# bioinfo-pf-curie/mpiBWA

Hardware: AMD Instinct MI355X
Metric: Mreads/s (whole node) 2x150 bp PE vs GRCh38-size reference; SAM bit-match (higher is better)
Workload: dtype int32

## Files before the change

mpibwa_amd/csrc/msw_kernel.hip:

```cpp
#include <hip/hip_runtime.h>
#include <type_traits>
#include "hip_util.h"
#include "device.h"

namespace mbw {

namespace {

#define MSW_PAD 7u

__device__ __forceinline__ int msw_base(const uint8_t *__restrict__ pac, int64_t l_pac, int64_t p)
{
	if (p >= l_pac) {
		int64_t f = (l_pac << 1) - 1 - p;
		return 3 - ((pac[f >> 2] >> ((~f & 3) << 1)) & 3);
	}
	return (pac[p >> 2] >> ((~p & 3) << 1)) & 3;
}

struct MswPassOut { int score, te, qe; };

#define MSW_QP(a, b, c, d) ((a) | (b) << 2 | (c) << 4 | (d) << 6)
template <int CTRL>
__device__ __forceinline__ int msw_dpp(int v) { return __builtin_amdgcn_update_dpp(0, v, CTRL, 0xf, 0xf, false); }

__device__ __forceinline__ uint32_t msw_code(const uint8_t *__restrict__ ms, int qlen, int is_rev, int k)
{
	if (k >= qlen) return MSW_PAD;
	if (is_rev) { const uint32_t b = ms[qlen - 1 - k]; return b < 4 ? 3 - b : 4; }
	const uint32_t c = ms[k];
	return c > 4 ? 4 : c;
}

__device__ __forceinline__ MswPassOut msw_pass(uint32_t *cell, const MswParams &P, const uint8_t *__restrict__ pac, bool live, int S, int tn,
                                               int64_t t0, int tdir, int endsc, int sat_limit, uint16_t *rows, size_t row_stride, int *sat_hit)
{
	const int lane = threadIdx.x, j = lane & 3;
	int gmax = 0, te = -1, qe = -1;
	bool run = live && tn > 0 && S > 0;
	const int oe_del = P.o_del + P.e_del, oe_ins = P.o_ins + P.e_ins, e_del = P.e_del, e_ins = P.e_ins;
	int Swave = run ? S : 0;
	for (int o = 32; o; o >>= 1) Swave = max(Swave, __shfl_xor(Swave, o));
	int co_diag = 0, co_fseg = 0, co_ffull = 0, co_key = 0;
	int tb_next = (run && j == 0) ? msw_base(pac, P.l_pac, t0) : 0;
	for (int t = 0; __any(run); ++t) {
		const int i = t - j;
		const bool act = run && i >= 0 && i < tn;
		const int tb = tb_next;
		if (run && i + 1 >= 0 && i + 1 < tn) tb_next = msw_base(pac, P.l_pac, t0 + (int64_t)(i + 1) * tdir);
		const uint32_t slo = tb == 0 ? P.slo[0] : tb == 1 ? P.slo[1] : tb == 2 ? P.slo[2] : P.slo[3];
		const uint32_t shi = (uint32_t)(uint8_t)(tb == 0 ? P.s4[0] : tb == 1 ? P.s4[1] : tb == 2 ? P.s4[2] : P.s4[3]);
		const int ci_diag = msw_dpp<MSW_QP(0, 0, 1, 2)>(co_diag), ci_fseg = msw_dpp<MSW_QP(0, 0, 1, 2)>(co_fseg);
		const int ci_ffull = msw_dpp<MSW_QP(0, 0, 1, 2)>(co_ffull), ci_key = msw_dpp<MSW_QP(0, 0, 1, 2)>(co_key);
		int diag = j ? ci_diag : 0, fseg = j ? ci_fseg : 0, ffull = j ? ci_ffull : 0;
		uint32_t key = j ? (uint32_t)ci_key : 0u;
		const int kbase = j * S;
		const int kmax = act ? S : 0;
		auto step = [&](uint32_t &w, int kk) {
			const int hk = w & 0x1fff;
			int e = (int)__builtin_amdgcn_ubfe(w, 13, 13);
			const uint32_t q = __builtin_amdgcn_ubfe(w, 26, 3);
			const int s = (int)(int8_t)__builtin_amdgcn_perm(shi, slo, q | 0x0c0c0c00u);
			const int h = max(max(diag + s, e), fseg);
			key = max(key, (uint32_t)h << 16 | (uint32_t)(0xffff - (kbase + kk)));
			const int hfin = max(h, ffull);
			e = max(max(e - e_del, h - oe_del), 0);
			const int t2 = h - oe_ins;
			fseg = max(max(fseg - e_ins, t2), 0);
			ffull = max(max(ffull - e_ins, t2), 0);
			fseg &= ~((int)w >> 31);
			diag = hk;
			w = (w & 0xfc000000u) | ((uint32_t)e << 13 | (uint32_t)hfin);
		};
		for (int k = 0; k < Swave; k += 2) {
			if (k < kmax) {
				uint32_t w0 = cell[k * 64 + lane], w1 = cell[(k + 1) * 64 + lane];
				step(w0, k); step(w1, k + 1);
				cell[k * 64 + lane] = w0; cell[(k + 1) * 64 + lane] = w1;
			}
		}
		if (act) { co_diag = diag; co_fseg = fseg; co_ffull = ffull; co_key = (int)key; }
		int stop = 0;
		if (act && j == 3) {
			const int imax = (int)(key >> 16);
			if (rows) rows[(size_t)i * row_stride] = (uint16_t)imax;
			if (imax > gmax) {
				gmax = imax; te = i; qe = 0xffff - (int)(key & 0xffff);
				if (gmax >= sat_limit) { *sat_hit = 1; stop = 1; }
				if (gmax >= endsc) stop = 1;
			}
			if (i + 1 >= tn) stop = 1;
		}
		stop = msw_dpp<MSW_QP(3, 3, 3, 3)>(stop);
		if (stop) run = false;
	}
	MswPassOut o;
	o.score = msw_dpp<MSW_QP(3, 3, 3, 3)>(gmax); o.te = msw_dpp<MSW_QP(3, 3, 3, 3)>(te); o.qe = msw_dpp<MSW_QP(3, 3, 3, 3)>(qe);
	*sat_hit = msw_dpp<MSW_QP(3, 3, 3, 3)>(*sat_hit);
	return o;
}

__device__ __forceinline__ void msw_tail(uint32_t *cell, const MswParams &P, const uint8_t *__restrict__ pac, bool live, const MswReq &rq, int qlen,
                                         const uint8_t *__restrict__ ms, int r, int n_req, MswPassOut f, int sat, uint16_t *__restrict__ rows,
                                         MswRes *__restrict__ res)
{
	const int lane = threadIdx.x, j = lane & 3;
	const int tlen = (int)(rq.re - rq.rb);
	const bool byte_flavour = qlen * P.a < 250;
	const int PP = byte_flavour ? 16 : 8;
	const int minsc = P.min_seed_len * P.a;
	const int sat_limit = byte_flavour ? 255 - P.shift : 0x10000;
	MswRes out;
	out.score = f.score; out.te = f.te; out.qe = f.qe; out.score2 = -1; out.te2 = -1; out.tb = -1; out.qb = -1; out.flags = sat;
	if (live && j == 0 && !sat && f.te >= 0 && f.score >= minsc) {
		const int d = (f.score + P.max_sc - 1) / P.max_sc;
		const int low = f.te - d, high = f.te + d;
		int last_sc = -1, last_i = -1;
		const int rows_done = f.te >= 0 ? tlen : 0;
		for (int i = 0; i < rows_done; ++i) {
			const int im = rows[(size_t)i * n_req + r];
			if (im < minsc) continue;
			if (last_i < 0 || last_i + 1 != i) {
				if (last_i >= 0 && (last_i < low || last_i > high) && last_sc > out.score2) { out.score2 = last_sc; out.te2 = last_i; }
				last_sc = im; last_i = i;
			} else if (last_sc < im) { last_sc = im; last_i = i; }
		}
		if (last_i >= 0 && (last_i < low || last_i > high) && last_sc > out.score2) { out.score2 = last_sc; out.te2 = last_i; }
	}
	const bool second = live && !sat && f.score >= minsc && f.qe >= 0 && f.te >= 0;
	int qlen2 = second ? f.qe + 1 : 0;
	if (second && f.qe >= qlen) qlen2 = 0;
	const int slen2 = (qlen2 + PP - 1) / PP, npos2 = slen2 * PP, S2 = npos2 >> 2;
	if (qlen2 > 0)
		for (int kk = 0; kk < S2; ++kk) {
			const int k = j * S2 + kk;
			const uint32_t c = k < qlen2 ? msw_code(ms, qlen, rq.is_rev, qlen2 - 1 - k) : MSW_PAD;
			cell[kk * 64 + lane] = c << 26 | ((k + 1) % slen2 == 0 ? 0x80000000u : 0u);
		}
	int sat2 = 0;
	MswPassOut g = msw_pass(cell, P, pac, qlen2 > 0, S2, f.te + 1, rq.rb + f.te, -1, f.score, sat_limit, nullptr, 0, &sat2);
	if (qlen2 > 0 && g.score == f.score) { out.tb = f.te - g.te; out.qb = f.qe - g.qe; }
	if (second && qlen2 == 0) out.flags = 1;
	if (sat2) out.flags = 1;
	if (live && j == 0) res[r] = out;
}

__global__ __launch_bounds__(64) void msw_kernel(MswParams P, int n_work, int n_req, const int *__restrict__ list, const MswReq *__restrict__ req,
                                                 const uint8_t *__restrict__ seq, const int64_t *__restrict__ off, const int *__restrict__ lens,
                                                 const uint8_t *__restrict__ pac, MswRes *__restrict__ res, uint16_t *__restrict__ rows)
{
	extern __shared__ uint32_t cell[];
	const int lane = threadIdx.x, j = lane & 3;
	const int slot = blockIdx.x * 16 + (lane >> 2);
	const bool live = slot < n_work;
	const int r = live ? (list ? list[slot] : slot) : 0;
	MswReq rq;
	rq.rb = rq.re = 0; rq.read = 0; rq.is_rev = 0;
	if (live) rq = req[r];
	const int qlen = live ? lens[rq.read] : 0;
	const int tlen = (int)(rq.re - rq.rb);
	const bool byte_flavour = qlen * P.a < 250;
	const int PP = byte_flavour ? 16 : 8;
	const int slen = (qlen + PP - 1) / PP;
	const int npos = slen * PP, S = npos >> 2;
	const uint8_t *ms = seq + (live ? off[rq.read] : 0);
	if (live)
		for (int kk = 0; kk < S; ++kk) {
			const int k = j * S + kk;
			cell[kk * 64 + lane] = msw_code(ms, qlen, rq.is_rev, k) << 26 | ((k + 1) % slen == 0 ? 0x80000000u : 0u);
		}
	const int sat_limit = byte_flavour ? 255 - P.shift : 0x10000;
	int sat = 0;
	MswPassOut f = msw_pass(cell, P, pac, live, S, tlen, rq.rb, 1, 0x10000, sat_limit, live ? rows + r : nullptr, (size_t)n_req, &sat);
	msw_tail(cell, P, pac, live, rq, qlen, ms, r, n_req, f, sat, rows, res);
}

typedef short msw_s2 __attribute__((ext_vector_type(2)));
__device__ __forceinline__ msw_s2 s2_of(uint32_t v) { return __builtin_bit_cast(msw_s2, v); }
__device__ __forceinline__ uint32_t u_of(msw_s2 v) { return __builtin_bit_cast(uint32_t, v); }
__device__ __forceinline__ msw_s2 s2_max(msw_s2 a, msw_s2 b) { return __builtin_elementwise_max(a, b); }
__device__ __forceinline__ msw_s2 s2_splat(int v) { msw_s2 r; r.x = (short)v; r.y = (short)v; return r; }
typedef unsigned short msw_u2 __attribute__((ext_vector_type(2)));
__device__ __forceinline__ msw_s2 s2_sub0(msw_s2 a, msw_s2 b)
{
	return __builtin_bit_cast(msw_s2, __builtin_elementwise_sub_sat(__builtin_bit_cast(msw_u2, a), __builtin_bit_cast(msw_u2, b)));
}

__device__ __forceinline__ int msw_tail_bucket(int score, int qe, int a)
{
	const int sb = score >= 80 * a ? 2 : score >= 40 * a ? 1 : 0;
	const int qb = qe >= 96 ? 2 : qe >= 48 ? 1 : 0;
	return sb * 3 + qb;
}

__device__ __forceinline__ uint32_t msw_slo(const MswParams &P, int t) { return t == 0 ? P.slo[0] : t == 1 ? P.slo[1] : t == 2 ? P.slo[2] : P.slo[3]; }
__device__ __forceinline__ int msw_s4(const MswParams &P, int t) { return t == 0 ? P.s4[0] : t == 1 ? P.s4[1] : t == 2 ? P.s4[2] : P.s4[3]; }

__global__ __launch_bounds__(64) void msw2_kernel(MswParams P, int n_pairs, int n_req, const int *__restrict__ pairs, const MswReq *__restrict__ req,
                                                  const uint8_t *__restrict__ seq, const int64_t *__restrict__ off, const int *__restrict__ lens,
                                                  const uint8_t *__restrict__ pac, MswRes *__restrict__ res, uint16_t *__restrict__ rows, int s_max,
                                                  int *__restrict__ tail_n, int *__restrict__ tail_list, int tail_cap)
{
	extern __shared__ uint32_t lds2[];
	uint32_t *cell = lds2;
	uint32_t *codes = lds2 + (size_t)s_max * 64;
	uint32_t *stab = codes + (size_t)((s_max + 7) >> 3) * 64;
	const int lane = threadIdx.x, j = lane & 3;
	for (int e = lane; e < 128; e += 64) {
		const int ta = e >> 5, tb = (e >> 3) & 3, q = e & 7;
		const int sa = q < 4 ? (int)(int8_t)(msw_slo(P, ta) >> (8 * q)) : q == 4 ? msw_s4(P, ta) : 0;
		const int sb = q < 4 ? (int)(int8_t)(msw_slo(P, tb) >> (8 * q)) : q == 4 ? msw_s4(P, tb) : 0;
		stab[e] = (uint32_t)(uint16_t)(int16_t)sa | (uint32_t)(uint16_t)(int16_t)sb << 16;
	}
	const int slot = blockIdx.x * 16 + (lane >> 2);
	const bool live = slot < n_pairs;
	const int rA = live ? pairs[2 * slot] : 0, rB = live ? pairs[2 * slot + 1] : -1;
	const bool hasB = rB >= 0;
	MswReq qa, qb;
	qa.rb = qa.re = 0; qa.read = 0; qa.is_rev = 0; qb = qa;
	if (live) { qa = req[rA]; if (hasB) qb = req[rB]; else { qb = qa; qb.re = qb.rb; } }
	const int qlen = live ? lens[qa.read] : 0;
	const int tnA = (int)(qa.re - qa.rb), tnB = (int)(qb.re - qb.rb);
	const int slen = (qlen + 15) / 16, npos = slen * 16, S = npos >> 2;
	const uint8_t *ms = seq + (live ? off[qa.read] : 0);
	if (live) {
		for (int kk = 0; kk < S; ++kk) cell[kk * 64 + lane] = 0;
		for (int c = 0; c * 8 < S; ++c) {
			uint32_t cd = 0;
			for (int u = 0; u < 8 && c * 8 + u < S; ++u) {
				const int k = j * S + c * 8 + u;
				cd |= (msw_code(ms, qlen, qa.is_rev, k) | ((k + 1) % slen == 0 ? 8u : 0u)) << (4 * u);
			}
			codes[c * 64 + lane] = cd;
		}
	}
	__builtin_amdgcn_fence(__ATOMIC_RELEASE, "wavefront");
	__builtin_amdgcn_wave_barrier();
	__builtin_amdgcn_fence(__ATOMIC_ACQUIRE, "wavefront");
	const int sat_limit = 255 - P.shift;
	int slen_u = 0;
	{
		const unsigned long long lv = __builtin_amdgcn_ballot_w64(live);
		if (lv) {
			const int first = __builtin_amdgcn_readlane(slen, __ffsll((long long)lv) - 1);
			slen_u = __builtin_amdgcn_ballot_w64(live && slen != first) ? 0 : first;
		}
	}
	int gmaxA = 0, teA = -1, qeA = -1, gmaxB = 0, teB = -1, qeB = -1, satA = 0, satB = 0;
	auto forward = [&](auto uniform_segments) {
		constexpr bool UNI = decltype(uniform_segments)::value;
		const int tn = tnA > tnB ? tnA : tnB;
		bool run = live && tn > 0 && S > 0;
		const msw_s2 oe_del = s2_splat(P.o_del + P.e_del), oe_ins = s2_splat(P.o_ins + P.e_ins), e_del = s2_splat(P.e_del), e_ins = s2_splat(P.e_ins);
		const msw_s2 zero = s2_splat(0);
		int Swave = run ? S : 0;
		for (int o = 32; o; o >>= 1) Swave = max(Swave, __shfl_xor(Swave, o));
		uint32_t co_diag = 0, co_fseg = 0, co_ffull = 0, co_key = 0;
		auto base_at = [&](const MswReq &rq, int tnx, int i) -> int {
			const int ii = i < tnx ? i : tnx - 1;
			return ii >= 0 ? msw_base(pac, P.l_pac, rq.rb + ii) : 0;
		};
		int ta_next = (run && j == 0) ? base_at(qa, tnA, 0) : 0, tb_next = (run && j == 0) ? base_at(qb, tnB, 0) : 0;
		uint16_t *rowsA = rows + rA, *rowsB = rows + (hasB ? rB : rA);
		for (int t = 0; __any(run); ++t) {
			const int i = t - j;
			const bool act = run && i >= 0 && i < tn;
			const int ta = ta_next, tb = tb_next;
			if (run && i + 1 >= 0 && i + 1 < tn) { ta_next = base_at(qa, tnA, i + 1); tb_next = base_at(qb, tnB, i + 1); }
			const uint32_t *srow = stab + ((ta << 2 | tb) << 3);
			const uint32_t ci_diag = (uint32_t)msw_dpp<MSW_QP(0, 0, 1, 2)>((int)co_diag), ci_fseg = (uint32_t)msw_dpp<MSW_QP(0, 0, 1, 2)>((int)co_fseg);
			const uint32_t ci_ffull = (uint32_t)msw_dpp<MSW_QP(0, 0, 1, 2)>((int)co_ffull);
			const uint32_t ci_key = (uint32_t)msw_dpp<MSW_QP(0, 0, 1, 2)>((int)co_key);
			msw_s2 diag = s2_of(j ? ci_diag : 0u), fseg = s2_of(j ? ci_fseg : 0u), ffull = s2_of(j ? ci_ffull : 0u);
			msw_u2 key = __builtin_bit_cast(msw_u2, j ? ci_key : 0u);
			msw_u2 c256 = {256, 256};
			asm volatile("" : "+v"(c256));
			msw_u2 poscv = {(unsigned short)(248 - j * S), (unsigned short)(248 - j * S)};
			const int kmax = act ? S : 0;
			auto step = [&](uint32_t &w, uint32_t cd, int u, bool seg_end, msw_u2 &mblk) {
				const msw_s2 hd = s2_of(__builtin_amdgcn_perm(0u, w, 0x0c020c00u));
				msw_s2 e = s2_of(__builtin_amdgcn_perm(0u, w, 0x0c030c01u));
				uint32_t q = __builtin_amdgcn_ubfe(cd, 4 * u, 3);
				asm("" : "+v"(q));
				const msw_s2 s = s2_of(srow[q]);
				const msw_s2 h = s2_max(s2_max(diag + s, e), fseg);
				const msw_u2 rel = {(unsigned short)(7 - u), (unsigned short)(7 - u)};
				mblk = __builtin_elementwise_max(mblk, __builtin_bit_cast(msw_u2, h) * c256 + rel);
				const msw_s2 hfin = s2_max(h, ffull);
				e = s2_max(s2_sub0(e, e_del), s2_sub0(h, oe_del));
				const msw_s2 t2 = s2_sub0(h, oe_ins);
				fseg = s2_max(s2_sub0(fseg, e_ins), t2);
				if constexpr (UNI) fseg = seg_end ? zero : fseg;
				else fseg = s2_of(u_of(fseg) & ~(uint32_t)__builtin_amdgcn_sbfe((int)cd, 4 * u + 3, 1));
				ffull = s2_max(s2_sub0(ffull, e_ins), t2);
				diag = hd;
				w = __builtin_amdgcn_perm(u_of(e), u_of(hfin), 0x06020400u);
			};
			int seg_pos = 0;
			const msw_u2 eight = {8, 8};
			for (int c = 0; c * 8 < Swave; ++c, poscv -= eight) {
				const uint32_t cd = c * 8 < kmax ? codes[c * 64 + lane] : 0u;
				msw_u2 mblk = {0, 0};
#pragma unroll
				for (int u = 0; u < 8; u += 2) {
					const int k = c * 8 + u;
					bool end0 = false, end1 = false;
					if constexpr (UNI) {
						end0 = ++seg_pos == slen_u; if (end0) seg_pos = 0;
						end1 = ++seg_pos == slen_u; if (end1) seg_pos = 0;
					}
					if (k < kmax) {
						uint32_t w0 = cell[k * 64 + lane], w1 = cell[(k + 1) * 64 + lane];
						step(w0, cd, u, end0, mblk); step(w1, cd, u + 1, end1, mblk);
						cell[k * 64 + lane] = w0; cell[(k + 1) * 64 + lane] = w1;
					}
				}
				if (c * 8 < kmax) key = __builtin_elementwise_max(key, mblk + poscv);
			}
			const uint32_t keyAB = __builtin_bit_cast(uint32_t, key);
			if (act) { co_diag = u_of(diag); co_fseg = u_of(fseg); co_ffull = u_of(ffull); co_key = keyAB; }
			int stop = 0;
			if (act && j == 3) {
				if (i < tnA && !satA) {
					const int imax = (int)(keyAB >> 8 & 0xff);
					rowsA[(size_t)i * n_req] = (uint16_t)imax;
					if (imax > gmaxA) { gmaxA = imax; teA = i; qeA = 255 - (int)(keyAB & 0xff); if (gmaxA >= sat_limit) satA = 1; }
				}
				if (i < tnB && !satB) {
					const int imax = (int)(keyAB >> 24);
					rowsB[(size_t)i * n_req] = (uint16_t)imax;
					if (imax > gmaxB) { gmaxB = imax; teB = i; qeB = 255 - (int)(keyAB >> 16 & 0xff); if (gmaxB >= sat_limit) satB = 1; }
				}
				if ((i + 1 >= tnA || satA) && (i + 1 >= tnB || satB)) stop = 1;
			}
			stop = msw_dpp<MSW_QP(3, 3, 3, 3)>(stop);
			if (stop) run = false;
		}
	};
	if (slen_u > 0) forward(std::true_type{}); else forward(std::false_type{});
	MswPassOut fA, fB;
	fA.score = msw_dpp<MSW_QP(3, 3, 3, 3)>(gmaxA); fA.te = msw_dpp<MSW_QP(3, 3, 3, 3)>(teA); fA.qe = msw_dpp<MSW_QP(3, 3, 3, 3)>(qeA);
	fB.score = msw_dpp<MSW_QP(3, 3, 3, 3)>(gmaxB); fB.te = msw_dpp<MSW_QP(3, 3, 3, 3)>(teB); fB.qe = msw_dpp<MSW_QP(3, 3, 3, 3)>(qeB);
	satA = msw_dpp<MSW_QP(3, 3, 3, 3)>(satA); satB = msw_dpp<MSW_QP(3, 3, 3, 3)>(satB);
	const int minsc = P.min_seed_len * P.a;
	const bool mineA = live && j == 0, mineB = live && hasB && j == 1;
	const MswPassOut f = j == 0 ? fA : fB;
	const int sat = j == 0 ? satA : satB;
	const bool tail = (mineA || mineB) && !sat && f.score >= minsc && f.qe >= 0 && f.te >= 0;
	if (mineA || mineB) {
		MswRes out;
		out.score = f.score; out.te = f.te; out.qe = f.qe; out.score2 = -1; out.te2 = -1; out.tb = -1; out.qb = -1; out.flags = sat;
		res[j == 0 ? rA : rB] = out;
	}
	const int bucket = msw_tail_bucket(f.score, f.qe, P.a);
#pragma unroll
	for (int b = 0; b < MSW_TAIL_BUCKETS; ++b) {
		const bool in = tail && bucket == b;
		const unsigned long long m = __builtin_amdgcn_ballot_w64(in);
		if (!m) continue;
		const int leader = __ffsll((long long)m) - 1;
		int at = 0;
		if (lane == leader) at = atomicAdd(&tail_n[b], __popcll(m));
		at = __shfl(at, leader);
		if (in) tail_list[(size_t)b * tail_cap + at + __popcll(m & ((1ull << lane) - 1))] = j == 0 ? rA : rB;
	}
}

__global__ __launch_bounds__(64) void msw_tail_kernel(MswParams P, int n_req, const int *__restrict__ tail_n, const int *__restrict__ tail_list, int tail_cap,
                                                      const MswReq *__restrict__ req, const uint8_t *__restrict__ seq, const int64_t *__restrict__ off,
                                                      const int *__restrict__ lens, const uint8_t *__restrict__ pac, MswRes *__restrict__ res,
                                                      const uint16_t *__restrict__ rows)
{
	extern __shared__ uint32_t lds_t[];
	uint16_t *blk = (uint16_t *)lds_t;
	uint32_t *cell = lds_t + 16 * 64 / 2;
	const int lane = threadIdx.x, j = lane & 3, quad = lane >> 2;
	int slot = blockIdx.x * 16 + quad, b = MSW_TAIL_BUCKETS - 1;
	for (; b >= 0; --b) {
		const int n = tail_n[b];
		if (slot < n) break;
		slot -= n;
	}
	const bool live = b >= 0;
	if (!__any(live)) return;
	const int r = live ? tail_list[(size_t)b * tail_cap + slot] : 0;
	MswReq rq;
	rq.rb = rq.re = 0; rq.read = 0; rq.is_rev = 0;
	MswRes out;
	out.score = 0; out.te = -1; out.qe = -1; out.score2 = -1; out.te2 = -1; out.tb = -1; out.qb = -1; out.flags = 0;
	if (live) { rq = req[r]; out = res[r]; }
	const int qlen = live ? lens[rq.read] : 0;
	const int tlen = live ? (int)(rq.re - rq.rb) : 0;
	const uint8_t *ms = seq + (live ? off[rq.read] : 0);
	const bool byte_flavour = qlen * P.a < 250;
	const int PP = byte_flavour ? 16 : 8;
	const int minsc = P.min_seed_len * P.a;
	const int sat_limit = byte_flavour ? 255 - P.shift : 0x10000;
	{
		const int d = (out.score + P.max_sc - 1) / P.max_sc;
		const int low = out.te - d, high = out.te + d;
		int last_sc = -1, last_i = -1, sc2 = -1, te2 = -1;
		int twave = tlen;
		for (int o = 32; o; o >>= 1) twave = max(twave, __shfl_xor(twave, o));
		uint16_t *qb = blk + quad * 64;
		for (int i0 = 0; i0 < twave; i0 += 64) {
			uint16_t v[16];
#pragma unroll
			for (int u = 0; u < 16; ++u) {
				const int i = i0 + u * 4 + j;
				v[u] = i < tlen ? rows[(size_t)i * n_req + r] : (uint16_t)0;
			}
			bool any = false;
#pragma unroll
			for (int u = 0; u < 16; ++u) {
				qb[u * 4 + j] = v[u];
				any |= i0 + u * 4 + j < tlen && (int)v[u] >= minsc;
			}
			if (!__any(any)) continue;
			__builtin_amdgcn_fence(__ATOMIC_RELEASE, "wavefront");
			__builtin_amdgcn_wave_barrier();
			__builtin_amdgcn_fence(__ATOMIC_ACQUIRE, "wavefront");
			const int kend = min(64, tlen - i0);
			for (int k = 0; k < kend; ++k) {
				const int i = i0 + k, im = qb[k];
				if (im < minsc) continue;
				if (last_i < 0 || last_i + 1 != i) {
					if (last_i >= 0 && (last_i < low || last_i > high) && last_sc > sc2) { sc2 = last_sc; te2 = last_i; }
					last_sc = im; last_i = i;
				} else if (last_sc < im) { last_sc = im; last_i = i; }
			}
			__builtin_amdgcn_fence(__ATOMIC_RELEASE, "wavefront");
			__builtin_amdgcn_wave_barrier();
			__builtin_amdgcn_fence(__ATOMIC_ACQUIRE, "wavefront");
		}
		if (last_i >= 0 && (last_i < low || last_i > high) && last_sc > sc2) { sc2 = last_sc; te2 = last_i; }
		out.score2 = sc2; out.te2 = te2;
	}
	int qlen2 = live ? out.qe + 1 : 0;
	if (live && out.qe >= qlen) qlen2 = 0;
	const int slen2 = (qlen2 + PP - 1) / PP, npos2 = slen2 * PP, S2 = npos2 >> 2;
	if (qlen2 > 0)
		for (int kk = 0; kk < S2; ++kk) {
			const int k = j * S2 + kk;
			const uint32_t c = k < qlen2 ? msw_code(ms, qlen, rq.is_rev, qlen2 - 1 - k) : MSW_PAD;
			cell[kk * 64 + lane] = c << 26 | ((k + 1) % slen2 == 0 ? 0x80000000u : 0u);
		}
	int sat2 = 0;
	const MswPassOut g = msw_pass(cell, P, pac, qlen2 > 0, S2, out.te + 1, rq.rb + out.te, -1, out.score, sat_limit, nullptr, 0, &sat2);
	if (qlen2 > 0 && g.score == out.score) { out.tb = out.te - g.te; out.qb = out.qe - g.qe; }
	if (live && qlen2 == 0) out.flags = 1;
	if (sat2) out.flags = 1;
	if (live && j == 0) res[r] = out;
}

}

size_t msw_lds_bytes(int max_len)
{
	return (size_t)((max_len + 15) / 16 * 16 / 4) * 64 * 4;
}

size_t msw2_lds_bytes(int max_len)
{
	const int s_max = (max_len + 15) / 16 * 16 / 4;
	return ((size_t)s_max * 64 + (size_t)((s_max + 7) / 8) * 64 + 128) * 4;
}

size_t msw_tail_lds_bytes(int max_len)
{
	return 16 * 64 * sizeof(uint16_t) + msw_lds_bytes(max_len);
}

static void msw_tail_census(void *stream, const MswParams &P, int n_req, int n_pairs, const int *h_list, const MswRes *d_res)
{
	std::vector<MswRes> res((size_t)n_req);
	HIP_OK(hipStreamSynchronize((hipStream_t)stream));
	HIP_OK(hipMemcpy(res.data(), d_res, (size_t)n_req * sizeof(MswRes), hipMemcpyDeviceToHost));
	const int minsc = P.min_seed_len * P.a;
	long hits_a = 0, hits_b = 0, waves_a = 0, waves_b = 0;
	for (int w = 0; w * 16 < n_pairs; ++w) {
		bool any_a = false, any_b = false;
		for (int s = w * 16; s < std::min(n_pairs, w * 16 + 16); ++s) {
			const int ra = h_list[2 * s], rb = h_list[2 * s + 1];
			if (res[ra].score >= minsc) { ++hits_a; any_a = true; }
			if (rb >= 0 && res[rb].score >= minsc) { ++hits_b; any_b = true; }
		}
		waves_a += any_a; waves_b += any_b;
	}
	fprintf(stderr, "[msw] packed work items: %ld + %ld alignments reach min_seed_len*a (%d); of %d waves, %ld hold an A hit, %ld a B hit\n", hits_a, hits_b,
	        minsc, (n_pairs + 15) / 16, waves_a, waves_b);
}

void launch_msw(void *stream, const MswParams &P, int n_req, const MswReq *d_req, const uint8_t *d_seq, const int64_t *d_off, const int *d_len,
                const uint8_t *d_pac, MswRes *d_res, uint16_t *d_rows, int max_len, const MswReq *h_req, const int *h_len, int *h_list, int *d_list,
                int *d_tail)
{
	if (n_req <= 0) return;
	const size_t lds = msw_lds_bytes(max_len), lds2 = msw2_lds_bytes(max_len), lds_t = msw_tail_lds_bytes(max_len);
	if (lds > 160 * 1024) die("mate-rescue kernel: reads of %d bp do not fit the LDS row buffers", max_len);
	static size_t s_attr = 0, s_attr2 = 0, s_attr_t = 0;
	if (lds > s_attr) {
		HIP_OK(hipFuncSetAttribute((const void *)msw_kernel, hipFuncAttributeMaxDynamicSharedMemorySize, (int)lds));
		s_attr = lds;
	}
	static const bool pairing = !(getenv("MPIBWA_MSW_PAIRS") && atoi(getenv("MPIBWA_MSW_PAIRS")) == 0);
	int n_pairs = 0, n_single = n_req;
	const int *d_single = nullptr;
	if (pairing && h_req && h_len && h_list && d_list && d_tail && lds2 <= 160 * 1024 && lds_t <= 160 * 1024) {
		int *pl = h_list, np = 0, ns = 0, n_alone = 0;
		int *sl_end = h_list + 2 * (size_t)n_req;
		for (int k = 0; k < n_req;) {
			const bool byte_k = h_len[h_req[k].read] * P.a < 250;
			if (!byte_k) { *--sl_end = k; ++ns; ++k; continue; }
			if (k + 1 < n_req && h_req[k].read == h_req[k + 1].read && h_req[k].is_rev == h_req[k + 1].is_rev && h_req[k].re > h_req[k].rb &&
			    h_req[k + 1].re > h_req[k + 1].rb) {
				pl[2 * np] = k; pl[2 * np + 1] = k + 1; ++np; k += 2;
			} else { pl[2 * np] = k; pl[2 * np + 1] = -1; ++np; ++n_alone; ++k; }
		}
		n_pairs = np; n_single = ns;
		static const bool say = getenv("MPIBWA_CPUSEC") != nullptr;
		if (say) fprintf(stderr, "[msw] %d requests: %d quads of two windows for one mate, %d of one, %d in the word flavour\n", n_req, np - n_alone, n_alone, ns);
		HIP_OK(hipMemcpyAsync(d_list, h_list, (size_t)2 * n_req * sizeof(int), hipMemcpyHostToDevice, (hipStream_t)stream));
		d_single = d_list + (sl_end - h_list);
		if (n_pairs) {
			if (lds2 > s_attr2) {
				HIP_OK(hipFuncSetAttribute((const void *)msw2_kernel, hipFuncAttributeMaxDynamicSharedMemorySize, (int)lds2));
				s_attr2 = lds2;
			}
			if (lds_t > s_attr_t) {
				HIP_OK(hipFuncSetAttribute((const void *)msw_tail_kernel, hipFuncAttributeMaxDynamicSharedMemorySize, (int)lds_t));
				s_attr_t = lds_t;
			}
			const int s_max = (max_len + 15) / 16 * 16 / 4;
			int *d_tail_n = d_tail, *d_tail_list = d_tail + 16;
			HIP_OK(hipMemsetAsync(d_tail_n, 0, MSW_TAIL_BUCKETS * sizeof(int), (hipStream_t)stream));
			hipLaunchKernelGGL(msw2_kernel, dim3((n_pairs + 15) / 16), dim3(64), lds2, (hipStream_t)stream, P, n_pairs, n_req, (const int *)d_list, d_req, d_seq, d_off,
			                   d_len, d_pac, d_res, d_rows, s_max, d_tail_n, d_tail_list, n_req);
			const int n_byte = 2 * n_pairs - n_alone;
			hipLaunchKernelGGL(msw_tail_kernel, dim3((n_byte + 15) / 16), dim3(64), lds_t, (hipStream_t)stream, P, n_req, (const int *)d_tail_n,
			                   (const int *)d_tail_list, n_req, d_req, d_seq, d_off, d_len, d_pac, d_res, (const uint16_t *)d_rows);
		}
	}
	if (n_single)
		hipLaunchKernelGGL(msw_kernel, dim3((n_single + 15) / 16), dim3(64), lds, (hipStream_t)stream, P, n_single, n_req, d_single, d_req, d_seq, d_off, d_len, d_pac,
		                   d_res, d_rows);
	HIP_OK(hipGetLastError());
	static const bool say = getenv("MPIBWA_CPUSEC") != nullptr;
	if (say && n_pairs) msw_tail_census(stream, P, n_req, n_pairs, h_list, d_res);
}

}
```

Before: 7.299.

## Keep mate-rescue SW row state in registers via slen-templated kernels

Result: faster. 7.787, median of 6 (+6.7%).

```diff
diff --git a/mpibwa_amd/csrc/msw_kernel.hip b/mpibwa_amd/csrc/msw_kernel.hip
--- a/mpibwa_amd/csrc/msw_kernel.hip
+++ b/mpibwa_amd/csrc/msw_kernel.hip
@@ -196,15 +196,17 @@
 __device__ __forceinline__ uint32_t msw_slo(const MswParams &P, int t) { return t == 0 ? P.slo[0] : t == 1 ? P.slo[1] : t == 2 ? P.slo[2] : P.slo[3]; }
 __device__ __forceinline__ int msw_s4(const MswParams &P, int t) { return t == 0 ? P.s4[0] : t == 1 ? P.s4[1] : t == 2 ? P.s4[2] : P.s4[3]; }
 
+template <int SLEN>
 __global__ __launch_bounds__(64) void msw2_kernel(MswParams P, int n_pairs, int n_req, const int *__restrict__ pairs, const MswReq *__restrict__ req,
                                                   const uint8_t *__restrict__ seq, const int64_t *__restrict__ off, const int *__restrict__ lens,
                                                   const uint8_t *__restrict__ pac, MswRes *__restrict__ res, uint16_t *__restrict__ rows, int s_max,
                                                   int *__restrict__ tail_n, int *__restrict__ tail_list, int tail_cap)
 {
+	constexpr bool REGS = SLEN > 0, TWO = REGS && SLEN < 16;
 	extern __shared__ uint32_t lds2[];
 	uint32_t *cell = lds2;
 	uint32_t *codes = lds2 + (size_t)s_max * 64;
-	uint32_t *stab = codes + (size_t)((s_max + 7) >> 3) * 64;
+	uint32_t *stab = REGS ? lds2 : codes + (size_t)((s_max + 7) >> 3) * 64;
 	const int lane = threadIdx.x, j = lane & 3;
 	for (int e = lane; e < 128; e += 64) {
 		const int ta = e >> 5, tb = (e >> 3) & 3, q = e & 7;
@@ -223,7 +225,21 @@
 	const int tnA = (int)(qa.re - qa.rb), tnB = (int)(qb.re - qb.rb);
 	const int slen = (qlen + 15) / 16, npos = slen * 16, S = npos >> 2;
 	const uint8_t *ms = seq + (live ? off[qa.read] : 0);
-	if (live) {
+	constexpr int RS = REGS ? 4 * SLEN : 1, RC = RS / 4 + (RS % 4 != 0);
+	uint32_t st0[RS], st1[TWO ? RS : 1], cdreg[RC];
+	if constexpr (REGS) {
+#pragma unroll
+		for (int kk = 0; kk < RS; ++kk) st0[kk] = 0;
+#pragma unroll
+		for (int kk = 0; kk < (TWO ? RS : 1); ++kk) st1[kk] = 0;
+#pragma unroll
+		for (int c = 0; c < RC; ++c) {
+			uint32_t cd = 0;
+#pragma unroll
+			for (int u = 0; u < 4; ++u) cd |= msw_code(ms, qlen, qa.is_rev, j * RS + c * 4 + u) << (8 * u + 2);
+			cdreg[c] = cd;
+		}
+	} else if (live) {
 		for (int kk = 0; kk < S; ++kk) cell[kk * 64 + lane] = 0;
 		for (int c = 0; c * 8 < S; ++c) {
 			uint32_t cd = 0;
@@ -337,7 +353,98 @@
 			if (stop) run = false;
 		}
 	};
-	if (slen_u > 0) forward(std::true_type{}); else forward(std::false_type{});
+	auto forward_regs = [&]() {
+		constexpr int S = RS, SL = REGS ? SLEN : 1;
+		const int tn = tnA > tnB ? tnA : tnB;
+		bool run = live && tn > 0;
+		const msw_s2 oe_del = s2_splat(P.o_del + P.e_del), oe_ins = s2_splat(P.o_ins + P.e_ins), e_del = s2_splat(P.e_del), e_ins = s2_splat(P.e_ins);
+		const msw_s2 zero = s2_splat(0);
+		uint32_t co_diag = 0, co_fseg = 0, co_ffull = 0, co_key = 0;
+		auto base_at = [&](const MswReq &rq, int tnx, int i) -> int {
+			const int ii = i < tnx ? i : tnx - 1;
+			return ii >= 0 ? msw_base(pac, P.l_pac, rq.rb + ii) : 0;
+		};
+		int ta_next = (run && j == 0) ? base_at(qa, tnA, 0) : 0, tb_next = (run && j == 0) ? base_at(qb, tnB, 0) : 0;
+		uint16_t *rowsA = rows + rA, *rowsB = rows + (hasB ? rB : rA);
+		const msw_u2 posc0 = {(unsigned short)(248 - j * S), (unsigned short)(248 - j * S)};
+		for (int t = 0; __any(run); ++t) {
+			const int i = t - j;
+			const bool act = run && i >= 0 && i < tn;
+			const int ta = ta_next, tb = tb_next;
+			if (run && i + 1 >= 0 && i + 1 < tn) { ta_next = base_at(qa, tnA, i + 1); tb_next = base_at(qb, tnB, i + 1); }
+			const uint32_t *srow = stab + ((ta << 2 | tb) << 3);
+			const uint32_t ci_diag = (uint32_t)msw_dpp<MSW_QP(0, 0, 1, 2)>((int)co_diag), ci_fseg = (uint32_t)msw_dpp<MSW_QP(0, 0, 1, 2)>((int)co_fseg);
+			const uint32_t ci_ffull = (uint32_t)msw_dpp<MSW_QP(0, 0, 1, 2)>((int)co_ffull);
+			const uint32_t ci_key = (uint32_t)msw_dpp<MSW_QP(0, 0, 1, 2)>((int)co_key);
+			if (act) {
+				msw_s2 diag = s2_of(j ? ci_diag : 0u), fseg = s2_of(j ? ci_fseg : 0u), ffull = s2_of(j ? ci_ffull : 0u);
+				msw_u2 key = __builtin_bit_cast(msw_u2, j ? ci_key : 0u);
+				msw_u2 c256 = {256, 256};
+				asm volatile("" : "+v"(c256));
+				auto lookups = [&](int c, uint32_t *sv) {
+#pragma unroll
+					for (int u = 0; u < 8 && c * 8 + u < S; ++u)
+						sv[u] = *(const uint32_t *)((const char *)srow + __builtin_amdgcn_ubfe(cdreg[(c * 8 + u) >> 2], 8 * (u & 3), 8));
+					__builtin_amdgcn_sched_barrier(0);
+				};
+				auto step = [&](int kk, int u, uint32_t sq, msw_u2 &mblk) {
+					msw_s2 hd, e;
+					if constexpr (TWO) { hd = s2_of(st0[kk]); e = s2_of(st1[kk]); }
+					else {
+						hd = s2_of(__builtin_amdgcn_perm(0u, st0[kk], 0x0c020c00u));
+						e = s2_of(__builtin_amdgcn_perm(0u, st0[kk], 0x0c030c01u));
+					}
+					const msw_s2 h = s2_max(s2_max(diag + s2_of(sq), e), fseg);
+					const msw_u2 rel = {(unsigned short)(7 - u), (unsigned short)(7 - u)};
+					mblk = __builtin_elementwise_max(mblk, __builtin_bit_cast(msw_u2, h) * c256 + rel);
+					const msw_s2 hfin = s2_max(h, ffull);
+					e = s2_max(s2_sub0(e, e_del), s2_sub0(h, oe_del));
+					const msw_s2 t2 = s2_sub0(h, oe_ins);
+					if ((kk + 1) % SL == 0) fseg = zero;
+					else fseg = s2_max(s2_sub0(fseg, e_ins), t2);
+					ffull = s2_max(s2_sub0(ffull, e_ins), t2);
+					diag = hd;
+					if constexpr (TWO) { st0[kk] = u_of(hfin); st1[kk] = u_of(e); }
+					else st0[kk] = __builtin_amdgcn_perm(u_of(e), u_of(hfin), 0x06020400u);
+				};
+				constexpr int NB = (S + 7) / 8;
+#pragma unroll
+				for (int c = 0; c < RC; ++c) asm volatile("" : "+v"(cdreg[c]));
+				uint32_t sv[2][8];
+				lookups(0, sv[0]);
+#pragma unroll
+				for (int c = 0; c < NB; ++c) {
+					if (c + 1 < NB) lookups(c + 1, sv[(c + 1) & 1]);
+					msw_u2 mblk = {0, 0};
+#pragma unroll
+					for (int u = 0; u < 8 && c * 8 + u < S; ++u) step(c * 8 + u, u, sv[c & 1][u], mblk);
+					const msw_u2 blk0 = {(unsigned short)(8 * c), (unsigned short)(8 * c)};
+					key = __builtin_elementwise_max(key, mblk + (posc0 - blk0));
+				}
+				co_diag = u_of(diag); co_fseg = u_of(fseg); co_ffull = u_of(ffull); co_key = __builtin_bit_cast(uint32_t, key);
+			}
+			const uint32_t keyAB = co_key;
+			int stop = 0;
+			if (act && j == 3) {
+				if (i < tnA && !satA) {
+					const int imax = (int)(keyAB >> 8 & 0xff);
+					rowsA[(size_t)i * n_req] = (uint16_t)imax;
+					if (imax > gmaxA) { gmaxA = imax; teA = i; qeA = 255 - (int)(keyAB & 0xff); if (gmaxA >= sat_limit) satA = 1; }
+				}
+				if (i < tnB && !satB) {
+					const int imax = (int)(keyAB >> 24);
+					rowsB[(size_t)i * n_req] = (uint16_t)imax;
+					if (imax > gmaxB) { gmaxB = imax; teB = i; qeB = 255 - (int)(keyAB >> 16 & 0xff); if (gmaxB >= sat_limit) satB = 1; }
+				}
+				if ((i + 1 >= tnA || satA) && (i + 1 >= tnB || satB)) stop = 1;
+			}
+			stop = msw_dpp<MSW_QP(3, 3, 3, 3)>(stop);
+			if (stop) run = false;
+		}
+	};
+	if constexpr (REGS) forward_regs();
+	else if (slen_u > 0) forward(std::true_type{});
+	else forward(std::false_type{});
 	MswPassOut fA, fB;
 	fA.score = msw_dpp<MSW_QP(3, 3, 3, 3)>(gmaxA); fA.te = msw_dpp<MSW_QP(3, 3, 3, 3)>(teA); fA.qe = msw_dpp<MSW_QP(3, 3, 3, 3)>(qeA);
 	fB.score = msw_dpp<MSW_QP(3, 3, 3, 3)>(gmaxB); fB.te = msw_dpp<MSW_QP(3, 3, 3, 3)>(teB); fB.qe = msw_dpp<MSW_QP(3, 3, 3, 3)>(qeB);
@@ -491,6 +598,15 @@
 	        minsc, (n_pairs + 15) / 16, waves_a, waves_b);
 }
 
+#define MSW_REGS_CLASSES 6
+static const int msw_regs_slen[MSW_REGS_CLASSES] = {5, 7, 8, 10, 13, 16};
+static int msw_regs_class(int slen)
+{
+	for (int c = 0; c < MSW_REGS_CLASSES; ++c)
+		if (msw_regs_slen[c] == slen) return c;
+	return MSW_REGS_CLASSES;
+}
+
 void launch_msw(void *stream, const MswParams &P, int n_req, const MswReq *d_req, const uint8_t *d_seq, const int64_t *d_off, const int *d_len,
                 const uint8_t *d_pac, MswRes *d_res, uint16_t *d_rows, int max_len, const MswReq *h_req, const int *h_len, int *h_list, int *d_list,
                 int *d_tail)
@@ -504,18 +620,41 @@
 		s_attr = lds;
 	}
 	static const bool pairing = !(getenv("MPIBWA_MSW_PAIRS") && atoi(getenv("MPIBWA_MSW_PAIRS")) == 0);
+	static const bool regs_form = !(getenv("MPIBWA_MSW_REGS") && atoi(getenv("MPIBWA_MSW_REGS")) == 0);
 	int n_pairs = 0, n_single = n_req;
 	const int *d_single = nullptr;
 	if (pairing && h_req && h_len && h_list && d_list && d_tail && lds2 <= 160 * 1024 && lds_t <= 160 * 1024) {
-		int *pl = h_list, np = 0, ns = 0, n_alone = 0;
+		int np = 0, ns = 0, n_alone = 0;
+		int cls_n[MSW_REGS_CLASSES + 1], cls_at[MSW_REGS_CLASSES + 1], order[MSW_REGS_CLASSES + 1];
 		int *sl_end = h_list + 2 * (size_t)n_req;
+		auto item = [&](int k, int &cls) -> int {
+			const int qlen = h_len[h_req[k].read];
+			if (!(qlen * P.a < 250)) return 0;
+			cls = regs_form ? msw_regs_class((qlen + 15) / 16) : MSW_REGS_CLASSES;
+			return k + 1 < n_req && h_req[k].read == h_req[k + 1].read && h_req[k].is_rev == h_req[k + 1].is_rev && h_req[k].re > h_req[k].rb &&
+			       h_req[k + 1].re > h_req[k + 1].rb ? 2 : 1;
+		};
+		for (int c = 0; c <= MSW_REGS_CLASSES; ++c) cls_n[c] = 0;
 		for (int k = 0; k < n_req;) {
-			const bool byte_k = h_len[h_req[k].read] * P.a < 250;
-			if (!byte_k) { *--sl_end = k; ++ns; ++k; continue; }
-			if (k + 1 < n_req && h_req[k].read == h_req[k + 1].read && h_req[k].is_rev == h_req[k + 1].is_rev && h_req[k].re > h_req[k].rb &&
-			    h_req[k + 1].re > h_req[k + 1].rb) {
-				pl[2 * np] = k; pl[2 * np + 1] = k + 1; ++np; k += 2;
-			} else { pl[2 * np] = k; pl[2 * np + 1] = -1; ++np; ++n_alone; ++k; }
+			int cls = 0;
+			const int w = item(k, cls);
+			if (w) ++cls_n[cls];
+			k += w ? w : 1;
+		}
+		for (int c = 0; c < MSW_REGS_CLASSES; ++c) order[c] = c;
+		for (int a = 1; a < MSW_REGS_CLASSES; ++a)
+			for (int b = a; b > 0 && cls_n[order[b]] > cls_n[order[b - 1]]; --b) std::swap(order[b], order[b - 1]);
+		order[MSW_REGS_CLASSES] = MSW_REGS_CLASSES;
+		for (int o = 0, at = 0; o <= MSW_REGS_CLASSES; ++o) { cls_at[order[o]] = at; at += cls_n[order[o]]; }
+		int cur[MSW_REGS_CLASSES + 1];
+		for (int c = 0; c <= MSW_REGS_CLASSES; ++c) cur[c] = cls_at[c];
+		for (int k = 0; k < n_req;) {
+			int cls = 0;
+			const int w = item(k, cls);
+			if (!w) { *--sl_end = k; ++ns; ++k; continue; }
+			int *pl = h_list + 2 * (size_t)cur[cls]++;
+			pl[0] = k; pl[1] = w == 2 ? k + 1 : -1;
+			++np; n_alone += w == 1; k += w;
 		}
 		n_pairs = np; n_single = ns;
 		static const bool say = getenv("MPIBWA_CPUSEC") != nullptr;
@@ -524,7 +663,7 @@
 		d_single = d_list + (sl_end - h_list);
 		if (n_pairs) {
 			if (lds2 > s_attr2) {
-				HIP_OK(hipFuncSetAttribute((const void *)msw2_kernel, hipFuncAttributeMaxDynamicSharedMemorySize, (int)lds2));
+				HIP_OK(hipFuncSetAttribute((const void *)msw2_kernel<0>, hipFuncAttributeMaxDynamicSharedMemorySize, (int)lds2));
 				s_attr2 = lds2;
 			}
 			if (lds_t > s_attr_t) {
@@ -534,8 +673,25 @@
 			const int s_max = (max_len + 15) / 16 * 16 / 4;
 			int *d_tail_n = d_tail, *d_tail_list = d_tail + 16;
 			HIP_OK(hipMemsetAsync(d_tail_n, 0, MSW_TAIL_BUCKETS * sizeof(int), (hipStream_t)stream));
-			hipLaunchKernelGGL(msw2_kernel, dim3((n_pairs + 15) / 16), dim3(64), lds2, (hipStream_t)stream, P, n_pairs, n_req, (const int *)d_list, d_req, d_seq, d_off,
-			                   d_len, d_pac, d_res, d_rows, s_max, d_tail_n, d_tail_list, n_req);
+			for (int o = 0; o <= MSW_REGS_CLASSES; ++o) {
+				const int c = order[o], n = cls_n[c];
+				if (!n) continue;
+				const int *d_items = d_list + 2 * (size_t)cls_at[c];
+				const dim3 grid((n + 15) / 16);
+#define MSW2_LAUNCH(SLEN) \
+	hipLaunchKernelGGL(msw2_kernel<SLEN>, grid, dim3(64), (SLEN) ? 128 * sizeof(uint32_t) : lds2, (hipStream_t)stream, P, n, n_req, d_items, d_req, d_seq, d_off, d_len, \
+	                   d_pac, d_res, d_rows, s_max, d_tail_n, d_tail_list, n_req)
+				switch (c < MSW_REGS_CLASSES ? msw_regs_slen[c] : 0) {
+				case 5: MSW2_LAUNCH(5); break;
+				case 7: MSW2_LAUNCH(7); break;
+				case 8: MSW2_LAUNCH(8); break;
+				case 10: MSW2_LAUNCH(10); break;
+				case 13: MSW2_LAUNCH(13); break;
+				case 16: MSW2_LAUNCH(16); break;
+				default: MSW2_LAUNCH(0);
+				}
+#undef MSW2_LAUNCH
+			}
 			const int n_byte = 2 * n_pairs - n_alone;
 			hipLaunchKernelGGL(msw_tail_kernel, dim3((n_byte + 15) / 16), dim3(64), lds_t, (hipStream_t)stream, P, n_req, (const int *)d_tail_n,
 			                   (const int *)d_tail_list, n_req, d_req, d_seq, d_off, d_len, d_pac, d_res, (const uint16_t *)d_rows);
```
